# zyddnys/sd_animation_optical_flow

Hardware: AMD Instinct MI355X
Metric: frame-pairs/sec (flow+warp+mask) at 512x768 (higher is better)
Workload: dtype f32

## Files before the change

include/ofx.h:

```cpp
#ifndef OFX_H
#define OFX_H

#include <stddef.h>
#include <stdint.h>

#ifdef __cplusplus
extern "C" {
#endif

#define OFX_VERSION 100

#define OFX_EINVAL   (-1)
#define OFX_EALIGN   (-2)
#define OFX_ENOMEM   (-3)
#define OFX_EKEY     (-4)
#define OFX_ENODEV   (-5)

int ofx_version(void);
const char* ofx_error_string(int code);

int ofx_prof_enable(int on);
int ofx_prof_collect(char* json_out, size_t cap);

#define OFX_WARP_BILINEAR  0
// ... 101 lines not shown
int ofx_clip_embed(const int32_t* ids, const float* tok, const float* pos, float* out, int ldo, long rows, int T, int C, int vocab,
                   void* stream);
int ofx_quick_gelu(const float* x, int ldx, float* out, int ldo, long rows, int n, void* stream);

typedef struct ofx_ddim_coef {
    float cfg, sqrt_at, sqrt_1m_at, sqrt_aprev, dir_coef, sigma_t, g, sa, s1;
} ofx_ddim_coef;
#define OFX_DDIM_STEP       0
#define OFX_DDIM_BLEND_ONLY 1
int ofx_ddim_step(const float* x, int ldx, const float* eps_c, const float* eps_u, int lde, const float* guidance, int ldg,
                  const float* gmap, const float* step_noise, int ldsn, const float* init, int ldi, const float* nmask, int ldm,
                  const float* blend_noise, int ldbn, float* out0, int ldo0, float* out1, int ldo1, float* pred_out, int ldp,
                  const ofx_ddim_coef* coef, int mode, long rows, int C, void* stream);

size_t ofx_detect_edges_scratch_bytes(int B, int H, int W);
int ofx_detect_edges(const uint8_t* frames_bgr, uint8_t* edges, void* scratch, size_t scratch_bytes, int B, int H,
                     int W, int ksize, void* stream);
size_t ofx_canny_u8_scratch_bytes(int B, int H, int W);
int ofx_canny_u8(const uint8_t* images, int channels, uint8_t* edges, void* scratch, size_t scratch_bytes, int B, int H,
                 int W, int low, int high, void* stream);
int ofx_abs_diff_sum_u8(const uint8_t* a, long a_bstride, const uint8_t* b, long b_bstride,
                        unsigned long long* sums, int B, long n, void* stream);

#define OFX_ACT_NONE    0
#define OFX_ACT_RELU    1
#define OFX_ACT_SIGMOID 2
#define OFX_ACT_TANH    3

#define OFX_EPI_PLAIN   0
#define OFX_EPI_GRU_ZR  1
#define OFX_EPI_GRU_Q   2
#define OFX_EPI_FLOW    3

#define OFX_PREC_FP32   0
#define OFX_PREC_BF16X3 1
#define OFX_PREC_BF16X3_W 2
#define OFX_PREC_BF16X6_W 4
#define OFX_PREC_BF16X6 3
#define OFX_PREC_F16 5
#define OFX_PREC_F16_EPI (OFX_PREC_F16 | 256)

typedef struct ofx_conv_desc {
    const float* in0; int ld0; int c0;
    const float* in1; int ld1; int c1;
    const float* w;
    const float* scale;
    const float* shift;
    float* out; int ldo;
    const float* res; int ldres;
    const float* nmean; const float* nrstd;
    const float* addend; int ldadd;
    float* aux_z; float* aux_rh; float* aux_h; int ldh;
    float* aux_coords; float* aux_flow4;
    long a_zs, w_zs, o_zs; int nz;
    int B, Hin, Win, Hout, Wout, Cout, KH, KW, stride, padH, padW;
    int act, epi;
    int tile;
    int precision;
    void* splitk_ws;
    size_t splitk_ws_bytes;
    const float* wino_w;
    const float* wino4_w;
} ofx_conv_desc;
#define OFX_CONV_TILE_WINOGRAD 1
#define OFX_CONV_TILE_WINOGRAD4 2

int ofx_conv2d(const ofx_conv_desc* d, void* stream);
typedef struct ofx_conv_plan {
    int path;
    int bm, bn, wm, wn, bk;
    int prec;
    int ks;
    int ksplit;
    int mode;
    int mtiles, ntiles, group_m;
    int stats_rows;
} ofx_conv_plan;
int ofx_conv2d_plan(const ofx_conv_desc* d, size_t stats_cap_floats, int want_pool, ofx_conv_plan* out);
long ofx_pack_conv_weight(const float* w_oihw, int Cout, int Cin, int KH, int KW, int cin_pad,
                          float* out);
int ofx_split_conv_weight(const float* packed, long n_floats, float* out);
long ofx_wino_conv_weight(const float* w_oihw, int Cout, int Cin, float* out);
long ofx_wino15_conv_weight(const float* w_oihw, int Cout, int Cin, int KH, int KW, float* out);
long ofx_wino44_conv_weight(const float* w_oihw, int Cout, int Cin, float* out);
int ofx_split_conv_weight3(const float* packed, long n_floats, float* out);

int ofx_inorm_stats(const float* x, int ld, float* mean, float* rstd, float* scratch,
                    int B, long HW, int C, float eps, void* stream);
int ofx_conv2d_stats(const ofx_conv_desc* d, float* part, size_t part_floats, int* rows_per_image, void* stream);
int ofx_inorm_finalize(const float* part, float* mean, float* rstd, int B, int rows, long HW, int C, float eps, void* stream);
int ofx_inorm_apply(const float* x, const float* mean, const float* rstd, const float* res,
                    const float* res_mean, const float* res_rstd, float* out, int B, long HW, int C,
                    int relu, void* stream);
int ofx_preprocess_u8(const uint8_t* img, float* out, long npix, int bgr, void* stream);

int ofx_corr_slice_floats(int h_l, int w_l);
int ofx_corr_volume(const float* f1, const float* f2, float* const* pyr, int B, int h, int w, int D,
                    int levels, void* stream);
int ofx_corr_volume_split(const float* f1, const float* f2, float* const* pyr, int B, int h, int w, int D,
                          int levels, int planes, int shared_f2, void* stream);
int ofx_corr_lookup(const float* const* pyr, const float* coords, float* out, int ldo, int B, int h,
                    int w, int levels, int radius, void* stream);
int ofx_local_corr_fwd(const float* fmap1, const float* fmap2, const float* coords, float* corr,
                       int B, int H1, int W1, int H2, int W2, int C, int N, int r, void* stream);
int ofx_local_corr_bwd(const float* fmap1, const float* fmap2, const float* coords, const float* corr_grad,
                       float* fmap1_grad, float* fmap2_grad, int B, int H1, int W1, int H2, int W2, int C, int N,
                       int r, void* stream);
int ofx_local_corr_rows(const float* fmap1, const float* const* fmap2_levels, const int* idx1, const int* idx2,
                        const float* coords, float* rows, int ld, int B, int H1, int W1, int C, int levels, int radius,
                        int tiled, void* stream);
int ofx_avgpool2_nhwc(const float* in, float* out, int B, int H, int W, int C, void* stream);

int ofx_upsample_flow(const float* coords1, const float* mask, float* flow_up, int B, int h, int w,
                      void* stream);
int ofx_upsample_flow_warp(const float* coords1, const float* mask, float* flow_up, const uint8_t* frame,
                           uint8_t* warped, int B, int h, int w, float sign, void* stream);
int ofx_upflow8(const float* coords1, float* flow_up, int B, int h, int w, void* stream);
int ofx_upflow8_warp(const float* coords1, float* flow_up, const uint8_t* frame, uint8_t* warped, int B, int h, int w,
                     float sign, void* stream);
int ofx_flow_head(const float* x, int ldx, const float* w, int kpad, const float* bias, float* coords1, float* hx_flow,
                  int ldh, float* frows, int B, int h, int w_, void* stream);

size_t ofx_forward_interpolate_scratch_bytes(int B, int h, int w);
int ofx_forward_interpolate(const float* flow, float* out, void* scratch, size_t scratch_bytes, int B, int h, int w, void* stream);

typedef struct ofx_tensor {
    const char* name;
    const float* data;
    int ndim; long shape[4];
} ofx_tensor;

typedef struct ofx_raft ofx_raft;

int ofx_raft_create(const ofx_tensor* tensors, int n, ofx_raft** out);
int ofx_raft_destroy(ofx_raft* r);
size_t ofx_raft_workspace_bytes(const ofx_raft* r, int B, int H, int W);
size_t ofx_raft_workspace_bytes_mode(const ofx_raft* r, int n_images, int B, int H, int W, int flags);

#define OFX_RAFT_BGR          1
#define OFX_RAFT_SHARED_IMG2  2
#define OFX_RAFT_SHARED_IMG1  4
#define OFX_RAFT_ALT_CORR     8
#define OFX_RAFT_BF16X3      16
#define OFX_RAFT_BF16X6      64
#define OFX_RAFT_BN_BATCH   128
#define OFX_RAFT_SEPARATE_STATS 256
#define OFX_RAFT_VOL_BF16X3  512
#define OFX_RAFT_VOL_BF16X6 1024
#define OFX_RAFT_SERIAL       32
#define OFX_RAFT_FLOW_INIT  2048
#define OFX_RAFT_F16 4096

int ofx_raft_forward(ofx_raft* r, const uint8_t* image1, const uint8_t* image2, int B, int H, int W,
                     int iters, int flags, float* flow_up, float* flow_low, void* workspace,
                     size_t workspace_bytes, void* stream);
int ofx_raft_forward_warp(ofx_raft* r, const uint8_t* image1, const uint8_t* image2, int B, int H, int W,
                          int iters, int flags, float* flow_up, float* flow_low, const uint8_t* warp_frame,
                          float warp_sign, uint8_t* warped, void* workspace, size_t workspace_bytes, void* stream);
size_t ofx_raft_workspace_bytes_pairs(const ofx_raft* r, int n_images, int B, int H, int W);
int ofx_raft_forward_pairs(ofx_raft* r, const uint8_t* images, int n_images, const int* idx1,
                           const int* idx2, int B, int H, int W, int iters, int flags, float* flow_up,
                           float* flow_low, void* workspace, size_t workspace_bytes, void* stream);
int ofx_raft_forward_pairs_warp(ofx_raft* r, const uint8_t* images, int n_images, const int* idx1,
                                const int* idx2, int B, int H, int W, int iters, int flags, float* flow_up,
                                float* flow_low, const uint8_t* warp_frame, float warp_sign, int n_warp,
                                uint8_t* warped, void* workspace, size_t workspace_bytes, void* stream);
// ... 8 lines not shown
```

sd_animation_optical_flow_amd/_lib.py:

```python
from __future__ import annotations

import ctypes as C
import os

_HERE = os.path.dirname(os.path.abspath(__file__))
LIB_PATH = os.environ.get("OFX_LIB_PATH") or os.path.join(_HERE, "libofx.so")


class OfxLibraryError(RuntimeError):
    pass


class OfxError(RuntimeError):
    def __init__(self, code: int, where: str):
        self.code = code
        super().__init__(f"{where}: {error_string(code)} (code {code})")


class ConvDesc(C.Structure):
    _fields_ = [
        ("in0", C.c_void_p), ("ld0", C.c_int), ("c0", C.c_int),
        ("in1", C.c_void_p), ("ld1", C.c_int), ("c1", C.c_int),
        ("w", C.c_void_p), ("scale", C.c_void_p), ("shift", C.c_void_p),
        ("out", C.c_void_p), ("ldo", C.c_int),
        ("res", C.c_void_p), ("ldres", C.c_int),
        ("nmean", C.c_void_p), ("nrstd", C.c_void_p),
        ("addend", C.c_void_p), ("ldadd", C.c_int),
        ("aux_z", C.c_void_p), ("aux_rh", C.c_void_p), ("aux_h", C.c_void_p), ("ldh", C.c_int),
        ("aux_coords", C.c_void_p), ("aux_flow4", C.c_void_p),
        ("a_zs", C.c_long), ("w_zs", C.c_long), ("o_zs", C.c_long), ("nz", C.c_int),
        ("B", C.c_int), ("Hin", C.c_int), ("Win", C.c_int), ("Hout", C.c_int), ("Wout", C.c_int),
        ("Cout", C.c_int), ("KH", C.c_int), ("KW", C.c_int), ("stride", C.c_int),
        ("padH", C.c_int), ("padW", C.c_int),
        ("act", C.c_int), ("epi", C.c_int), ("tile", C.c_int), ("precision", C.c_int),
        ("splitk_ws", C.c_void_p), ("splitk_ws_bytes", C.c_size_t),
        ("wino_w", C.c_void_p),
        ("wino4_w", C.c_void_p),
    ]


class ConvPlan(C.Structure):
    _fields_ = [(n, C.c_int) for n in ("path", "bm", "bn", "wm", "wn", "bk", "prec", "ks", "ksplit", "mode", "mtiles", "ntiles",
                                       "group_m", "stats_rows")]


class MaskRoute(C.Structure):
    _fields_ = [(n, C.c_int) for n in ("kernel", "band_rows", "threads", "nplanes", "xcd_map", "lds_bytes", "workgroups")]


class DdimCoef(C.Structure):
    _fields_ = [(n, C.c_float) for n in ("cfg", "sqrt_at", "sqrt_1m_at", "sqrt_aprev", "dir_coef", "sigma_t", "g", "sa", "s1")]


class Tensor(C.Structure):
    _fields_ = [("name", C.c_char_p), ("data", C.c_void_p), ("ndim", C.c_int), ("shape", C.c_long * 4)]


_p, _i, _l, _f, _z = C.c_void_p, C.c_int, C.c_long, C.c_float, C.c_size_t

SIGNATURES = {
    "ofx_version": (_i, []),
    "ofx_error_string": (C.c_char_p, [_i]),
    "ofx_prof_enable": (_i, [_i]),
    "ofx_prof_collect": (_i, [C.c_char_p, _z]),
    "ofx_warp_u8": (_i, [_p, _l, _p, _p, _i, _i, _i, _i, _i, _f, _p]),
    "ofx_warp_f32": (_i, [_p, _l, _p, _p, _i, _i, _i, _i, _i, _f, _p]),
    "ofx_resize_cubic_f32": (_i, [_p, _p, _i, _i, _i, _i, _i, _i, _p]),
    "ofx_generate_mask": (_i, [_p, _p, _p, _i, _i, _i, _f, _i, _i, _p]),
    "ofx_dilate_u8": (_i, [_p, _p, _i, _i, _i, _i, _p]),
    "ofx_expand_mask": (_i, [_p, _p, _p, _p, _i, _i, _i, _i, _i, _p]),
    "ofx_mask_plan": (_i, [_i, _i, _i, _i, _i, _i, C.POINTER(MaskRoute)]),
    "ofx_travel_distance": (_i, [_p, _p, _p, _i, _i, _i, _f, _p]),
    "ofx_flow_magnitude": (_i, [_p, _p, _l, _p]),
    "ofx_travel_mask": (_i, [_p, _p, _p, _p, _p, _p, _i, _i, _i, _f, _i, _p]),
    "ofx_merge_images": (_i, [_p, _p, _p, _p, _i, _i, _i, _i, _p]),
    "ofx_mix_frames": (_i, [_p, _p, _p, _p, _i, _i, _i, _i, _f, _p]),
    "ofx_conf_sum": (_i, [_p, _p, _i, _l, _i, _i, _p]),
    "ofx_fb_confidence": (_i, [_p, _p, _p, _p, _i, _i, _i, _f, _p]),
    "ofx_warp_and_mask": (_i, [_p, _l, _p, _p, _p, _p, _i, _i, _i, _i, _i, _f, _f, _i, _i, _p]),
    "ofx_compose_scratch_bytes": (_z, [_i, _i, _i]),
    "ofx_compose_refs": (_i, [_p] * 9 + [_z, _i, _i, _i, _f, _i, _i, _p]),
    "ofx_conv2d": (_i, [C.POINTER(ConvDesc), _p]),
    "ofx_conv2d_plan": (_i, [C.POINTER(ConvDesc), _z, _i, C.POINTER(ConvPlan)]),
    "ofx_pack_conv_weight": (_l, [_p, _i, _i, _i, _i, _i, _p]),
    "ofx_wino_conv_weight": (_l, [_p, _i, _i, _p]),
    "ofx_wino15_conv_weight": (_l, [_p, _i, _i, _i, _i, _p]),
    "ofx_wino44_conv_weight": (_l, [_p, _i, _i, _p]),
    "ofx_split_conv_weight": (_i, [_p, _l, _p]),
    "ofx_split_conv_weight3": (_i, [_p, _l, _p]),
    "ofx_gaussian_blur_u8": (_i, [_p, _p, _p, _i, _i, _i, _f, _p]),
    "ofx_resize_bicubic_u8": (_i, [_p, _p, _p, _i, _i, _i, _i, _i, _p]),
    "ofx_sd_handoff": (_i, [_p] * 9 + [_i] * 5 + [_p]),
    "ofx_gaussian_blur_rgba_u8": (_i, [_p, _p, _p, _i, _i, _i, _f, _p]),
    "ofx_fill_mask_input_scratch_bytes": (_z, [_i, _i, _i]),
    "ofx_fill_mask_input": (_i, [_p, _p, _p, _p, _i, _i, _i, _p]),
    "ofx_detect_edges_scratch_bytes": (_z, [_i, _i, _i]),
    "ofx_detect_edges": (_i, [_p, _p, _p, _z, _i, _i, _i, _i, _p]),
    "ofx_canny_u8_scratch_bytes": (_z, [_i, _i, _i]),
    "ofx_canny_u8": (_i, [_p, _i, _p, _p, _z, _i, _i, _i, _i, _i, _p]),
    "ofx_abs_diff_sum_u8": (_i, [_p, _l, _p, _l, _p, _i, _l, _p]),
    "ofx_inorm_stats": (_i, [_p, _i, _p, _p, _p, _i, _l, _i, _f, _p]),
    "ofx_conv2d_stats": (_i, [C.POINTER(ConvDesc), _p, _z, _p, _p]),
    "ofx_inorm_finalize": (_i, [_p, _p, _p, _i, _i, _l, _i, _f, _p]),
    "ofx_inorm_apply": (_i, [_p, _p, _p, _p, _p, _p, _p, _i, _l, _i, _i, _p]),
    "ofx_preprocess_u8": (_i, [_p, _p, _l, _i, _p]),
    "ofx_groupnorm_scratch_bytes": (C.c_size_t, [_i, _i]),
    "ofx_groupnorm": (_i, [_p, _p, _p, _p, _p, C.c_size_t, _i, C.c_long, _i, _i, C.c_float, _i, _p]),
    "ofx_softmax_rows": (_i, [_p, C.c_long, C.c_long, _i, C.c_float, _p, C.c_long, C.c_long, _p]),
    "ofx_attention_workspace_bytes": (C.c_size_t, [_i, _i, _i, _i]),
    "ofx_attention_f32": (_i, [_p, _p, _p, _p, C.c_long, _p, _i, _i, _i, _i, C.c_float, _p, C.c_size_t, _p]),
    "ofx_attention_prec": (_i, [_p, _p, _p, _p, C.c_long, _p, _i, _i, _i, _i, C.c_float, _i, _p, C.c_size_t, _p]),
    "ofx_layernorm": (_i, [_p, _i, _p, _p, _p, _i, _i, _i, _f, _p]),
    "ofx_geglu": (_i, [_p, _i, _p, _i, _i, _i, _p]),
    "ofx_attention_bnhd_f32": (_i, [_p, _i, _p, _i, _p, _i, _p, _l, _p, _i, _i, _i, _i, _i, _i, _f, _p]),
    "ofx_attention_bnhd_prec": (_i, [_p, _i, _p, _i, _p, _i, _p, _l, _p, _i, _i, _i, _i, _i, _i, _f, _i, _p]),
    "ofx_upconv2x_weight": (_l, [_p, _i, _i, _p]),
    "ofx_upconv2x": (_i, [_p, _p, _p, _p, _i, _i, _i, _i, _i, _i, _p]),
    "ofx_upsample2x_nearest_f32": (_i, [_p, _p, _i, _i, _i, _i, _p]),
    "ofx_decode_to_u8": (_i, [_p, _i, _p, _i, _i, _i, _p]),
    "ofx_groupnorm_cat_scratch_bytes": (_z, [_i, _i]),
    "ofx_groupnorm_cat": (_i, [_p, _i, _i, _p, _i, _i, _p, _i, _p, _p, _p, _p, _z, _i, _l, _i, _f, _i, _p]),
    "ofx_emb_linear": (_i, [_p, _i, _p, _p, _p, _i, _i, _i, _i, _i, _p]),
    "ofx_timestep_embedding": (_i, [_p, _p, _p, _i, _i, _p]),
    "ofx_ddim_step": (_i, [_p, _i, _p, _p, _i, _p, _i, _p, _p, _i, _p, _i, _p, _i, _p, _i, _p, _i, _p, _i, _p, _i, C.POINTER(DdimCoef), _i, _l, _i, _p]),
    "ofx_conv3x3_silu": (_i, [_p, _i, _i, _p, _i, _p, _p, _i, _i, _i, _i, _i, _i, _i, _p]),
    "ofx_clip_embed": (_i, [_p, _p, _p, _p, _i, _l, _i, _i, _i, _p]),
    "ofx_quick_gelu": (_i, [_p, _i, _p, _i, _l, _i, _p]),
    "ofx_corr_slice_floats": (_i, [_i, _i]),
    "ofx_corr_volume": (_i, [_p, _p, C.POINTER(_p), _i, _i, _i, _i, _i, _p]),
    "ofx_corr_volume_split": (_i, [_p, _p, C.POINTER(_p), _i, _i, _i, _i, _i, _i, _i, _p]),
    "ofx_corr_lookup": (_i, [C.POINTER(_p), _p, _p, _i, _i, _i, _i, _i, _i, _p]),
    "ofx_local_corr_fwd": (_i, [_p, _p, _p, _p, _i, _i, _i, _i, _i, _i, _i, _i, _p]),
    "ofx_local_corr_bwd": (_i, [_p] * 6 + [_i] * 8 + [_p]),
    "ofx_local_corr_rows": (_i, [_p] * 6 + [_i] * 8 + [_p]),
    "ofx_avgpool2_nhwc": (_i, [_p, _p, _i, _i, _i, _i, _p]),
    "ofx_upsample_flow": (_i, [_p, _p, _p, _i, _i, _i, _p]),
    "ofx_upsample_flow_warp": (_i, [_p, _p, _p, _p, _p, _i, _i, _i, _f, _p]),
    "ofx_upflow8": (_i, [_p, _p, _i, _i, _i, _p]),
    "ofx_upflow8_warp": (_i, [_p, _p, _p, _p, _i, _i, _i, _f, _p]),
    "ofx_flow_head": (_i, [_p, _i, _p, _i, _p, _p, _p, _i, _p, _i, _i, _i, _p]),
    "ofx_forward_interpolate_scratch_bytes": (_z, [_i, _i, _i]),
    "ofx_forward_interpolate": (_i, [_p, _p, _p, _z, _i, _i, _i, _p]),
    "ofx_raft_create": (_i, [C.POINTER(Tensor), _i, C.POINTER(_p)]),
    "ofx_raft_destroy": (_i, [_p]),
    "ofx_raft_workspace_bytes": (_z, [_p, _i, _i, _i]),
    "ofx_raft_workspace_bytes_mode": (_z, [_p, _i, _i, _i, _i, _i]),
    "ofx_raft_forward": (_i, [_p, _p, _p, _i, _i, _i, _i, _i, _p, _p, _p, _z, _p]),
    "ofx_raft_forward_warp": (_i, [_p, _p, _p, _i, _i, _i, _i, _i, _p, _p, _p, _f, _p, _p, _z, _p]),
    "ofx_raft_workspace_bytes_pairs": (_z, [_p, _i, _i, _i, _i]),
    "ofx_raft_forward_pairs": (_i, [_p, _p, _i, C.POINTER(_i), C.POINTER(_i), _i, _i, _i, _i, _i, _p, _p, _p, _z, _p]),
    "ofx_raft_forward_pairs_warp": (_i, [_p, _p, _i, C.POINTER(_i), C.POINTER(_i), _i, _i, _i, _i, _i, _p, _p, _p, _f, _i, _p, _p, _z, _p]),
    "ofx_raft_variant": (_i, [_p]),
    "ofx_raft_buffer": (_i, [_p, C.c_char_p, C.POINTER(_p), C.POINTER(_z)]),
}

_lib = None


def lib() -> C.CDLL:
    global _lib
    if _lib is not None:
        return _lib
    if not os.path.exists(LIB_PATH):
        raise OfxLibraryError(
            f"{LIB_PATH} not found: the HIP library has not been built. There is no CPU fallback; "
            "run `python -c 'import __graft_entry__ as g; g.build()'` at the repo root.")
    try:
        handle = C.CDLL(LIB_PATH)
    except OSError as e:
# ... 20 lines not shown
```

sd_animation_optical_flow_amd/csrc/conv_wino.hip:

```cpp
#include "ofx_internal.h"

#include <cmath>
#include <cstdlib>
#include <cstring>

namespace {

constexpr int kWBK = 16;
constexpr int kLDV = kWBK + 4;
constexpr int kOOB = 0x7FFFFFF0;

template <int W_, int H_, int Y0, int X0> struct HaloGeom {
    static constexpr int W = W_, H = H_, y_org = Y0, x_org = X0;
    static constexpr int pix = W * H;
    static constexpr int items = pix * (kWBK / 4);
    static constexpr int slots = (items + 255) / 256;
};
template <bool VERT> struct Halo15 : HaloGeom<VERT ? 16 : 20, VERT ? 12 : 8, VERT ? -2 : 0, VERT ? 0 : -2> {
    static constexpr int ldh = VERT ? 16 : 20;
    static constexpr int floats = Halo15::pix * ldh;
    __device__ static int at(int pix) { return pix * ldh; }
};
struct Halo3x3 : HaloGeom<18, 10, -1, -1> {
    static constexpr int lpair = 36, lrow = 336;
    static constexpr int floats = H * lrow;
    __device__ static int at(int y, int x) { return y * lrow + (x >> 1) * lpair + (x & 1) * 16; }
    __device__ static int at(int pix) { return at(pix / W, pix % W); }
};

struct WinoK {
    const float* in0;
    const float* in1;
    const float* u;
    const float* scale;
    const float* shift;
    const float* addend;
    const float* res;
    const float* nmean;
    const float* nrstd;
    float* stats;
    float* out;
    float* aux_z;
    float* aux_rh;
    float* aux_h;
    int ld0, c0, ld1, cin, ldo, ldadd, ldh, ldres;
    int H, W, Cout, act;
    int nblk;
    int nb32;
    int tpr, tpi, mtiles;
    int bytes0, bytes1, bytesu;
    float alpha;
    int vec4;
};

struct Patch {
    int nb, pb, y0, x0;
};

template <int PH = 8, int PW = 16> __device__ __forceinline__ Patch wino_patch(const WinoK& p) {
    const int nblk = p.mtiles * p.nblk;
    const int bid = blockIdx.x;
    const int q8 = nblk >> 3, r8 = nblk & 7;
    const int xcd = bid & 7, idx = bid >> 3;
    const int L = (xcd < r8 ? xcd * (q8 + 1) : r8 * (q8 + 1) + (xcd - r8) * q8) + idx;
    const int nb = L % p.nblk, mt = L / p.nblk;
    const int pb = mt / p.tpi;
    const int trem = mt - pb * p.tpi;
    const int py = trem / p.tpr;
    return {nb, pb, py * PH, (trem - py * p.tpr) * PW};
}

typedef int v4i __attribute__((ext_vector_type(4)));

template <class HALO, bool NORM> struct HaloStage {
    const WinoK& p;
    const int pb, tid;
    const float* in1s;
    int bytes1s;
    int hpix[HALO::slots];
    unsigned hok = 0;
    int hq;
    struct Regs {
        float4 pa[HALO::slots];
        float4 pmu, prs;
    } own;

    __device__ __forceinline__ HaloStage(const WinoK& p_, const Patch& pt, int tid_) : p(p_), pb(pt.pb), tid(tid_) {
        in1s = p.in1 ? p.in1 : p.in0;
        bytes1s = p.in1 ? p.bytes1 : p.bytes0;
#pragma unroll
        for (int k = 0; k < HALO::slots; ++k) {
            const int i = tid + 256 * k;
            const int pix = i >> 2;
            const int hy = pix / HALO::W, hx = pix - hy * HALO::W;
            const int gy = pt.y0 + HALO::y_org + hy, gx = pt.x0 + HALO::x_org + hx;
            const bool ok = i < HALO::items && (unsigned)gy < (unsigned)p.H && (unsigned)gx < (unsigned)p.W;
            hpix[k] = ok ? (pt.pb * p.H + gy) * p.W + gx : 0;
            hok |= (ok ? 1u : 0u) << k;
        }
        hq = (tid & 3) * 16;
    }
    __device__ __forceinline__ void issue(int cb) { issue(cb, own); }
    __device__ __forceinline__ void store(float* Hs) const { store(Hs, own); }
    __device__ __forceinline__ void issue(int cb, Regs& r) {
        const int c = cb * kWBK;
        const bool s0 = c < p.c0;
        const __amdgpu_buffer_rsrc_t rs = __builtin_amdgcn_make_buffer_rsrc((void*)(s0 ? p.in0 : in1s), (short)0, s0 ? p.bytes0 : bytes1s, 0x00020000);
        const int so = (s0 ? c : c - p.c0) * 4;
        const int ldb = (s0 ? p.ld0 : p.ld1) * 4;
#pragma unroll
        for (int k = 0; k < HALO::slots; ++k) {
            const int vo = ((hok >> k) & 1u) ? hpix[k] * ldb + hq : kOOB;
            v4i t = __builtin_amdgcn_raw_buffer_load_b128(rs, vo, so, 0);
            r.pa[k] = *reinterpret_cast<float4*>(&t);
        }
        if constexpr (NORM) {
            const long at = (long)pb * p.c0 + c + (tid & 3) * 4;
            r.pmu = *reinterpret_cast<const float4*>(p.nmean + at);
            r.prs = *reinterpret_cast<const float4*>(p.nrstd + at);
        }
    }
    __device__ __forceinline__ void store(float* Hs, const Regs& r) const {
#pragma unroll
        for (int k = 0; k < HALO::slots; ++k) {
            const int i = tid + 256 * k;
            if (HALO::slots * 256 > HALO::items && k == HALO::slots - 1 && i >= HALO::items) break;
            float4 v = r.pa[k];
            if constexpr (NORM) {
                v.x = fmaxf((v.x - r.pmu.x) * r.prs.x, 0.f);
                v.y = fmaxf((v.y - r.pmu.y) * r.prs.y, 0.f);
                v.z = fmaxf((v.z - r.pmu.z) * r.prs.z, 0.f);
                v.w = fmaxf((v.w - r.pmu.w) * r.prs.w, 0.f);
                if (!((hok >> k) & 1u)) v = make_float4(0.f, 0.f, 0.f, 0.f);
            }
            *reinterpret_cast<float4*>(&Hs[HALO::at(i >> 2) + (i & 3) * 4]) = v;
// ... 271 lines not shown
            const int tile = (e & 3) + 8 * (e >> 2) + 4 * (lane >> 5);
            const float m0 = acc[0][nt][e], m1 = acc[1][nt][e], m2 = acc[2][nt][e], m3 = acc[3][nt][e];
            X[((wave * 2 + 0) * 32 + tile) * kLDX + (lane & 31)] = m0 + m1 + m2;
            X[((wave * 2 + 1) * 32 + tile) * kLDX + (lane & 31)] = m1 - m2 - m3;
        }
        __syncthreads();
        const int oc = pt.nb * 64 + nt * 32 + on;
        if (oc < p.Cout) {
            const float sc = (p.scale ? p.scale[oc] : 1.0f) * p.alpha;
            const float sh = p.shift ? p.shift[oc] : 0.0f;
            float st_s = 0.0f, st_q = 0.0f;
#pragma unroll
            for (int ty = 0; ty < 4; ++ty) {
                const int tile = ty * 8 + otx;
                float x[4][2];
#pragma unroll
                for (int w = 0; w < 4; ++w)
#pragma unroll
                    for (int j = 0; j < 2; ++j) x[w][j] = X[((w * 2 + j) * 32 + tile) * kLDX + on];
                float r[2][2];
                if constexpr (RES) {
#pragma unroll
                    for (int a = 0; a < 2; ++a)
#pragma unroll
                        for (int j = 0; j < 2; ++j)
                            r[a][j] = p.res[(((long)pt.pb * p.H + pt.y0 + 2 * ty + a) * p.W + pt.x0 + 2 * otx + j) * p.ldres + oc];
                }
#pragma unroll
                for (int a = 0; a < 2; ++a)
#pragma unroll
                    for (int j = 0; j < 2; ++j) {
                        const float y = a == 0 ? x[0][j] + x[1][j] + x[2][j] : x[1][j] - x[2][j] - x[3][j];
                        const long pix = ((long)pt.pb * p.H + pt.y0 + 2 * ty + a) * p.W + pt.x0 + 2 * otx + j;
                        float v = fmaxf(y * sc + sh, act_lo);
                        if constexpr (RES) v = fmaxf(v + r[a][j], 0.0f);
                        p.out[pix * p.ldo + oc] = v;
                        if constexpr (STATS) {
                            st_s += v;
                            st_q = fmaf(v, v, st_q);
                        }
                    }
            }
            if constexpr (STATS) {
                st_s += __shfl_xor(st_s, 32, 64);
                st_q += __shfl_xor(st_q, 32, 64);
                if (lane < 32) {
                    Sx[((nt * 4 + wave) * 32 + on) * 2 + 0] = st_s;
                    Sx[((nt * 4 + wave) * 32 + on) * 2 + 1] = st_q;
                }
            }
        }
    }
    if constexpr (STATS) {
        __syncthreads();
        const int nt = tid >> 5;
        const int oc = pt.nb * 64 + nt * 32 + on;
        if (tid < 64 && oc < p.Cout) {
            float s = 0.0f, q = 0.0f;
#pragma unroll
            for (int w = 0; w < 4; ++w) {
                s += Sx[((nt * 4 + w) * 32 + on) * 2 + 0];
                q += Sx[((nt * 4 + w) * 32 + on) * 2 + 1];
            }
            const long row = (long)pt.pb * p.tpi + (pt.y0 >> 3) * p.tpr + (pt.x0 >> 4);
            p.stats[(row * p.Cout + oc) * 2 + 0] = s;
            p.stats[(row * p.Cout + oc) * 2 + 1] = q;
        }
    }
}

template <bool VERT, int EPI>
__global__ __launch_bounds__(256, 2) void wino15_conv_kernel(const WinoK p) {
    using T = Wino15<VERT>;
    using HALO = typename T::HALO;
    __shared__ __attribute__((aligned(16))) float smem[HALO::floats + 8 * 32 * kLDV];
    float* const Hs = smem;
    float* const Vs = smem + HALO::floats;
    const int tid = threadIdx.x, lane = tid & 63;
    const int wave = __builtin_amdgcn_readfirstlane(tid >> 6);
    const Patch pt = wino_patch(p);
    f32x16 acc[8][1];
    wino_slabs_staged<T>(p, pt, Hs, Vs, tid, wave, acc);

    const int n = pt.nb * 128 + wave * 32 + (lane & 31);
    if (n >= p.Cout) return;
    const float sc = (p.scale ? p.scale[n] : 1.0f) * p.alpha;
    const float sh = p.shift ? p.shift[n] : 0.0f;
    const float act_lo = p.act == OFX_ACT_RELU ? 0.0f : -3.402823466e38f;
    const int hd = p.Cout >> 1;
    const bool r_half = EPI == OFX_EPI_GRU_ZR && pt.nb * 128 >= hd;
#pragma unroll
    for (int eb = 0; eb < 16; eb += 4) {
        long pix[4][4];
        float y[4][4], ad[4][4], x1[4][4], x2[4][4];
#pragma unroll
        for (int u = 0; u < 4; ++u) {
            const int e = eb + u;
            const int tile = (e & 3) + 8 * (e >> 2) + 4 * (lane >> 5);
#pragma unroll
            for (int i = 0; i < 4; ++i) pix[u][i] = ((long)pt.pb * p.H + pt.y0 + T::oy(tile, i)) * p.W + pt.x0 + T::ox(tile, i);
            const float m0 = acc[0][0][e], m1 = acc[1][0][e], m2 = acc[2][0][e], m3 = acc[3][0][e];
            const float m4 = acc[4][0][e], m5 = acc[5][0][e], m6 = acc[6][0][e], m7 = acc[7][0][e];
            const float s12 = m1 + m2, d12 = m1 - m2, s34 = m3 + m4, d34 = m3 - m4, s56 = m5 + m6, d56 = m5 - m6;
            y[u][0] = m0 + s12 + s34 + s56;
            y[u][1] = d12 + 2.0f * d34 + 0.5f * d56;
            y[u][2] = s12 + 4.0f * s34 + 0.25f * s56;
            y[u][3] = d12 + 8.0f * d34 + 0.125f * d56 + m7;
        }
#pragma unroll
        for (int u = 0; u < 4; ++u)
#pragma unroll
            for (int i = 0; i < 4; ++i) {
                ad[u][i] = p.addend ? p.addend[pix[u][i] * p.ldadd + n] : 0.0f;
                x1[u][i] = EPI == OFX_EPI_GRU_ZR ? (r_half ? p.aux_h[pix[u][i] * p.ldh + n - hd] : 1.0f)
                           : EPI == OFX_EPI_GRU_Q ? p.aux_z[pix[u][i] * p.Cout + n] : 0.0f;
                x2[u][i] = EPI == OFX_EPI_GRU_Q ? p.aux_h[pix[u][i] * p.ldh + n] : 0.0f;
            }
#pragma unroll
        for (int u = 0; u < 4; ++u)
#pragma unroll
            for (int i = 0; i < 4; ++i) {
                const float v = y[u][i] * sc + sh + ad[u][i];
                if (EPI == OFX_EPI_PLAIN) {
                    p.out[pix[u][i] * p.ldo + n] = fmaxf(v, act_lo);
                } else if (EPI == OFX_EPI_GRU_ZR) {
                    const float g = ofx_sigmoid(v) * x1[u][i];
                    if (r_half) p.aux_rh[pix[u][i] * hd + n - hd] = g;
                    else p.aux_z[pix[u][i] * hd + n] = g;
                } else {
                    p.aux_h[pix[u][i] * p.ldh + n] = (1.0f - x1[u][i]) * x2[u][i] + x1[u][i] * ofx_tanh(v);
                }
            }
    }
}

struct Halo44 {
    static constexpr int W = 34, H = 18;
    static constexpr int lquad = 34, lrow = 308;
    static constexpr int floats = H * lrow;
    static constexpr int items = W * H * 2;
    static constexpr int threads = 768;
    static constexpr int slots = (items + threads - 1) / threads;
    __device__ __host__ static constexpr int at(int y, int x) { return y * lrow + (x >> 2) * lquad + (x & 3) * 8; }
    static constexpr int ltrow = 336;
    static constexpr int tfloats = 6 * 4 * ltrow;
    static constexpr int titems = 4 * W * 4;
};
constexpr int kLDX4 = 40;
constexpr int kXF4 = 12 * 4 * 16 * kLDX4;
constexpr int kStage44 = 2 * (Halo44::floats + Halo44::tfloats);
constexpr int kSmem44 = (kStage44 > kXF4 ? kStage44 : kXF4) * 4;
constexpr int kNorm44 = kSmem44 / 4 - kStage44;
constexpr int kNorm44MaxCin = kNorm44 / 2 / kWBK * kWBK;
constexpr int kSX4 = 2 * 48 * 32 * 2;
static_assert(kNorm44 >= 0 && kSX4 <= kXF4, "the fused options live in the plain kernel's LDS");

__global__ __launch_bounds__(768, 1) void wino44_conv_kernel(const WinoK p) {
    extern __shared__ __attribute__((aligned(16))) float smem44[];
    constexpr bool NORM = false, RES = false, STATS = false;
#include "conv_wino44_body.inl"
}

template <bool NORM, bool RES, bool STATS>
__global__ __launch_bounds__(768, 1) void wino44_fused_kernel(const WinoK p) {
    extern __shared__ __attribute__((aligned(16))) float smem44[];
#include "conv_wino44_body.inl"
}


using WinoKernel = void (*)(WinoK);

const WinoKernel kKernels22[8] = {wino_conv_kernel<false, false, false>, wino_conv_kernel<false, false, true>,
                                  wino_conv_kernel<false, true, false>,  nullptr,
                                  wino_conv_kernel<true, false, false>,  wino_conv_kernel<true, false, true>,
                                  wino_conv_kernel<true, true, false>,   nullptr};
const WinoKernel kKernels15[8] = {wino15_conv_kernel<true, OFX_EPI_PLAIN>,  wino15_conv_kernel<true, OFX_EPI_GRU_ZR>,
                                  wino15_conv_kernel<true, OFX_EPI_GRU_Q>,  wino15_conv_kernel<false, OFX_EPI_PLAIN>,
                                  wino15_conv_kernel<false, OFX_EPI_GRU_ZR>, wino15_conv_kernel<false, OFX_EPI_GRU_Q>,
                                  nullptr,                                  nullptr};
const WinoKernel kKernels44[8] = {wino44_conv_kernel,                       wino44_fused_kernel<false, false, true>,
                                  wino44_fused_kernel<false, true, false>,  nullptr,
                                  wino44_fused_kernel<true, false, false>,  wino44_fused_kernel<true, false, true>,
                                  wino44_fused_kernel<true, true, false>,   nullptr};

struct WinoAlg {
    bool one_d;
    int ph, pw;
    int points, outputs;
    int cblk;
    int threads, dyn_lds;
    const float* ofx_conv_desc::*u;
    int tile;
    long min_grid;
    bool per_block;
    bool gates;
    bool norm_pair;
    int norm_max_cin;
    int path, path_fused;
    const WinoKernel* kernels;
};

const WinoAlg kAlgs[] = {
    {false, 16, 32, 36, 16, 64, 768, kSmem44, &ofx_conv_desc::wino4_w, OFX_CONV_TILE_WINOGRAD4, 768, true,
     false, true, kNorm44MaxCin, kPathWino44, kPathWino44Fused, kKernels44},
    {false, 8, 16, 16, 4, 64, 256, 0, &ofx_conv_desc::wino_w, OFX_CONV_TILE_WINOGRAD, 1024, true,
     false, false, 0x7FFFFFFF, kPathWino3x3, kPathWino3x3, kKernels22},
    {true, 8, 16, 8, 4, 128, 256, 0, &ofx_conv_desc::wino_w, OFX_CONV_TILE_WINOGRAD, 256, false,
     true, false, 0, kPathWino15, kPathWino15, kKernels15},
};
constexpr int kNumAlgs = sizeof kAlgs / sizeof kAlgs[0];

bool is_1d(int KH, int KW) { return (KH == 1 && KW == 5) || (KH == 5 && KW == 1); }

bool wino_fits(const WinoAlg& a, const ofx_conv_desc* d) {
    const int cin = d->c0 + d->c1;
    const float* const u = d->*a.u;
    const bool plain = d->epi == OFX_EPI_PLAIN && d->out != nullptr && d->ldo >= d->Cout && (d->act == OFX_ACT_NONE || d->act == OFX_ACT_RELU);
    const bool shape = a.one_d ? is_1d(d->KH, d->KW) : d->KH == 3 && d->KW == 3;
    bool epi;
    if (a.gates) {
        epi = !d->nmean && !d->res && (plain || (d->epi == OFX_EPI_GRU_ZR && (d->Cout / 2) % a.cblk == 0) || d->epi == OFX_EPI_GRU_Q);
    } else {
        epi = plain && !d->addend && (!d->res || d->ldres >= d->Cout) && (!a.norm_pair || (d->nmean != nullptr) == (d->nrstd != nullptr)) &&
              (!d->nmean || (d->nrstd && !d->in1 && d->c0 <= a.norm_max_cin && ofx_aligned16(d->nmean) && ofx_aligned16(d->nrstd)));
    }
    return shape && epi && d->padH == d->KH / 2 && d->padW == d->KW / 2 && d->precision == OFX_PREC_FP32 && d->nz <= 1 && d->stride == 1 &&
           d->Hout == d->Hin && d->Wout == d->Win && d->Hin % a.ph == 0 && d->Win % a.pw == 0 && cin % kWBK == 0 && d->c0 % kWBK == 0 &&
           u != nullptr && ofx_aligned16(u);
}

int wino_stats_rows(const WinoAlg& a, const ofx_conv_desc* d) {
    return !a.gates && d->act == OFX_ACT_NONE && !d->res ? (d->Hin / a.ph) * (d->Win / a.pw) : 0;
}

int wino_args(const WinoAlg& a, const ofx_conv_desc* d, float alpha, float* stats, WinoK* out) {
    WinoK k{};
    k.in0 = d->in0; k.in1 = d->in1; k.u = d->*a.u; k.scale = d->scale; k.shift = d->shift; k.addend = d->addend; k.out = d->out;
    k.res = d->res; k.nmean = d->nmean; k.nrstd = d->nrstd; k.stats = stats;
    k.aux_z = d->aux_z; k.aux_rh = d->aux_rh; k.aux_h = d->aux_h;
    k.ld0 = d->ld0; k.c0 = d->c0; k.ld1 = d->ld1; k.cin = d->c0 + d->c1; k.ldo = d->ldo; k.ldadd = d->ldadd; k.ldh = d->ldh;
    k.ldres = d->ldres;
    k.H = d->Hin; k.W = d->Win; k.Cout = d->Cout; k.act = d->act;
    k.nblk = (d->Cout + a.cblk - 1) / a.cblk;
    k.nb32 = a.cblk / 32 * k.nblk;
    k.tpr = d->Win / a.pw;
    k.tpi = (d->Hin / a.ph) * k.tpr;
    const long mtiles = (long)d->B * k.tpi;
    const long npix = (long)d->B * d->Hin * d->Win;
    const long ext0 = ((npix - 1) * d->ld0 + d->c0) * 4, ext1 = d->in1 ? ((npix - 1) * d->ld1 + d->c1) * 4 : 0;
    const long extu = (long)a.points * k.nb32 * 32 * k.cin * 4;
    OFX_REQUIRE(ext0 < (1L << 31) - 64 && ext1 < (1L << 31) - 64 && extu < (1L << 31) - 64, OFX_EINVAL);
    OFX_REQUIRE(mtiles * k.nblk < (1L << 31) && (a.one_d || npix * d->ldo < (1L << 31)), OFX_EINVAL);
    k.mtiles = (int)mtiles;
    k.bytes0 = (int)ext0; k.bytes1 = (int)ext1; k.bytesu = (int)extu;
    k.alpha = alpha;
    k.vec4 = ofx_aligned16(d->out) && d->ldo % 4 == 0 && ofx_aligned16(d->scale) && ofx_aligned16(d->shift) &&
             (!d->res || (ofx_aligned16(d->res) && d->ldres % 4 == 0));
    *out = k;
    return 0;
}

int wino_launch_kernel(const WinoAlg& a, int v, const WinoK& k, hipStream_t s, hipEvent_t stop_event) {
    const WinoKernel kernel = v >= 0 && v < 8 ? a.kernels[v] : nullptr;
    OFX_REQUIRE(kernel != nullptr, OFX_EINVAL);
    if (a.dyn_lds > 65536) {
        static bool allowed[64][kNumAlgs][8] = {};
        int dev = 0;
        if (hipGetDevice(&dev) != hipSuccess || dev < 0 || dev >= 64) return OFX_EINVAL;
        bool& ok = allowed[dev][&a - kAlgs][v];
        if (!ok) {
            const hipError_t e = hipFuncSetAttribute(reinterpret_cast<const void*>(kernel), hipFuncAttributeMaxDynamicSharedMemorySize, a.dyn_lds);
            if (e != hipSuccess) return (int)e;
            ok = true;
        }
    }
    const dim3 grid((unsigned)(k.mtiles * k.nblk), 1, 1), block(a.threads, 1, 1);
    if (stop_event) hipExtLaunchKernelGGL(kernel, grid, block, a.dyn_lds, s, nullptr, stop_event, 0, k);
    else hipLaunchKernelGGL(kernel, grid, block, a.dyn_lds, s, k);
    return ofx_launch_status();
}

}

int ofx_conv_wino_choose(const ofx_conv_desc* d, bool want_stats, size_t stats_cap, bool pool, bool no_wino, bool no_wino15, bool no_wino44,
                         OfxWinoChoice* c) {
    *c = OfxWinoChoice{};
    const bool off[kNumAlgs] = {no_wino44, no_wino, no_wino15};
    const bool one_d = is_1d(d->KH, d->KW);
    for (int i = 0; i < kNumAlgs; ++i) {
        const WinoAlg& a = kAlgs[i];
        const bool force = d->tile == a.tile;
        if (a.one_d != one_d || !(force || (d->tile == 0 && !off[i] && d->*a.u))) continue;
        const int srows = want_stats ? wino_stats_rows(a, d) : 0;
        const bool stats_ok = !want_stats || (srows > 0 && (size_t)d->B * srows * d->Cout * 2 <= stats_cap);
        if (!(stats_ok && !pool && wino_fits(a, d))) continue;
        const long patches = (long)d->B * (d->Hin / a.ph) * (d->Win / a.pw);
        if (!force && patches * (a.per_block ? (d->Cout + a.cblk - 1) / a.cblk : 1) < a.min_grid) continue;
        c->path = want_stats || d->res || d->nmean || d->nrstd ? a.path_fused : a.path;
        c->stats_rows = srows;
        c->flops = 2.0 * a.points * ((double)d->B * d->Hout * d->Wout / a.outputs) * (double)(d->c0 + d->c1) * d->Cout;
        return 0;
    }
    return d->tile == OFX_CONV_TILE_WINOGRAD || d->tile == OFX_CONV_TILE_WINOGRAD4 ? OFX_EINVAL : 0;
}

int ofx_conv_wino_launch(const ofx_conv_desc* d, int path, float alpha, float* stats, hipStream_t s, hipEvent_t stop_event) {
    const WinoAlg* a = nullptr;
    for (const WinoAlg& row : kAlgs)
        if (path == row.path || path == row.path_fused) a = &row;
    OFX_REQUIRE(a && (!stats || wino_stats_rows(*a, d) > 0), OFX_EINVAL);
    WinoK k;
    if (int st = wino_args(*a, d, alpha, stats, &k)) return st;
    const int v = a->gates ? (d->epi >= OFX_EPI_PLAIN && d->epi <= OFX_EPI_GRU_Q ? (d->KH == 5 ? 0 : 3) + d->epi : -1)
                           : (k.nmean ? 4 : 0) | (k.res ? 2 : 0) | (k.stats ? 1 : 0);
    return wino_launch_kernel(*a, v, k, s, stop_event);
}

namespace {

template <class XF>
long wino_weight(const float* w, int Cout, int Cin, int taps, int points, int cblk, float* out, XF xf) {
    OFX_REQUIRE(Cout > 0 && Cin > 0 && Cin % kWBK == 0, OFX_EINVAL);
    const int nb32 = cblk / 32 * ((Cout + cblk - 1) / cblk);
    const long n = (long)points * nb32 * 32 * Cin;
    if (!out) return n;
    OFX_REQUIRE(w != nullptr, OFX_EINVAL);
    std::memset(out, 0, (size_t)n * sizeof(float));
    double u[16];
    for (int o = 0; o < Cout; ++o)
        for (int c = 0; c < Cin; ++c) {
            xf(w + ((size_t)o * Cin + c) * taps, u);
            for (int q = 0; q < points; ++q) {
                const long at = ((((long)q * nb32 + o / 32) * (Cin / 8) + c / 8) * 2 + (c % 8) / 4) * 128 + 4 * (o % 32) + c % 4;
                out[at] = (float)u[q];
            }
        }
    return n;
}

}

extern "C" long ofx_wino_conv_weight(const float* w, int Cout, int Cin, float* out) {
    return wino_weight(w, Cout, Cin, 9, 16, 64, out, [](const float* g, double* u) {
        static const double G[4][3] = {{1, 0, 0}, {0.5, 0.5, 0.5}, {0.5, -0.5, 0.5}, {0, 0, 1}};
        double gg[4][3];
        for (int i = 0; i < 4; ++i)
            for (int x = 0; x < 3; ++x) gg[i][x] = G[i][0] * g[x] + G[i][1] * g[3 + x] + G[i][2] * g[6 + x];
        for (int i = 0; i < 4; ++i)
            for (int j = 0; j < 4; ++j) u[4 * i + j] = gg[i][0] * G[j][0] + gg[i][1] * G[j][1] + gg[i][2] * G[j][2];
    });
}

extern "C" long ofx_wino15_conv_weight(const float* w, int Cout, int Cin, int KH, int KW, float* out) {
    OFX_REQUIRE(is_1d(KH, KW), OFX_EINVAL);
    return wino_weight(w, Cout, Cin, 5, 8, 128, out, [](const float* g, double* u) {
        static const double G[8][5] = {
            {1, 0, 0, 0, 0},
            {-2.0 / 9, -2.0 / 9, -2.0 / 9, -2.0 / 9, -2.0 / 9},
            {-2.0 / 9, 2.0 / 9, -2.0 / 9, 2.0 / 9, -2.0 / 9},
            {1.0 / 90, 1.0 / 45, 2.0 / 45, 4.0 / 45, 8.0 / 45},
            {1.0 / 90, -1.0 / 45, 2.0 / 45, -4.0 / 45, 8.0 / 45},
            {32.0 / 45, 16.0 / 45, 8.0 / 45, 4.0 / 45, 2.0 / 45},
            {32.0 / 45, -16.0 / 45, 8.0 / 45, -4.0 / 45, 2.0 / 45},
            {0, 0, 0, 0, 1},
        };
        for (int q = 0; q < 8; ++q) {
            u[q] = 0.0;
            for (int t = 0; t < 5; ++t) u[q] += G[q][t] * (double)g[t];
        }
    });
}

extern "C" long ofx_wino44_conv_weight(const float* w, int Cout, int Cin, float* out) {
    OFX_REQUIRE(Cout > 0 && Cin > 0 && Cin % kWBK == 0, OFX_EINVAL);
    const int nb32 = 2 * ((Cout + 63) / 64);
    const long n = 36L * nb32 * 32 * Cin;
    if (!out) return n;
    OFX_REQUIRE(w != nullptr, OFX_EINVAL);
    std::memset(out, 0, (size_t)n * sizeof(float));
    static const double G[6][3] = {{1.0 / 4, 0, 0},           {-1.0 / 6, -1.0 / 6, -1.0 / 6}, {-1.0 / 6, 1.0 / 6, -1.0 / 6},
                                   {1.0 / 24, 1.0 / 12, 1.0 / 6}, {1.0 / 24, -1.0 / 12, 1.0 / 6}, {0, 0, 1}};
    for (int o = 0; o < Cout; ++o)
        for (int c = 0; c < Cin; ++c) {
            const float* g = w + ((size_t)o * Cin + c) * 9;
            double gg[6][3];
            for (int i = 0; i < 6; ++i)
                for (int x = 0; x < 3; ++x) gg[i][x] = G[i][0] * g[x] + G[i][1] * g[3 + x] + G[i][2] * g[6 + x];
            for (int i = 0; i < 6; ++i)
                for (int j = 0; j < 6; ++j) {
                    const double u = gg[i][0] * G[j][0] + gg[i][1] * G[j][1] + gg[i][2] * G[j][2];
                    const long q = 6 * i + j;
                    const long at = ((((q * nb32 + o / 32) * (Cin / 8) + c / 8) * 2 + (c % 4) / 2) * 2 + (c % 8) / 4) * 64 + 2 * (o % 32) + c % 2;
                    out[at] = (float)u;
                }
        }
    return n;
}
```

Baseline: 373.9.

## Transpose wino15 gated epilogue through LDS for vectorized float4 channel stores

The Winograd 1x5/5x1 gated-conv epilogue (plain, GRU z/r, GRU q) used to have each lane write one channel to scattered pixels with scalar loads and stores. It now stages each wave's output tile through LDS so every lane holds four consecutive channels of one pixel, then does float4 loads of addend and aux tensors and float4 stores. A host-side alignment check picks the vector path and keeps a scalar tail for partial quads. This should cut memory transactions on the epilogue, at the cost of LDS traffic, wave barriers and extra code complexity.

```diff
diff --git a/include/ofx.h b/include/ofx.h
--- a/include/ofx.h
+++ b/include/ofx.h
@@ -207,6 +207,7 @@
 int ofx_split_conv_weight(const float* packed, long n_floats, float* out);
 long ofx_wino_conv_weight(const float* w_oihw, int Cout, int Cin, float* out);
 long ofx_wino15_conv_weight(const float* w_oihw, int Cout, int Cin, int KH, int KW, float* out);
+int ofx_conv_wino15_vec(const ofx_conv_desc* d);
 long ofx_wino44_conv_weight(const float* w_oihw, int Cout, int Cin, float* out);
 int ofx_split_conv_weight3(const float* packed, long n_floats, float* out);
 
diff --git a/sd_animation_optical_flow_amd/_lib.py b/sd_animation_optical_flow_amd/_lib.py
--- a/sd_animation_optical_flow_amd/_lib.py
+++ b/sd_animation_optical_flow_amd/_lib.py
@@ -85,6 +85,7 @@
     "ofx_pack_conv_weight": (_l, [_p, _i, _i, _i, _i, _i, _p]),
     "ofx_wino_conv_weight": (_l, [_p, _i, _i, _p]),
     "ofx_wino15_conv_weight": (_l, [_p, _i, _i, _i, _i, _p]),
+    "ofx_conv_wino15_vec": (_i, [C.POINTER(ConvDesc)]),
     "ofx_wino44_conv_weight": (_l, [_p, _i, _i, _p]),
     "ofx_split_conv_weight": (_i, [_p, _l, _p]),
     "ofx_split_conv_weight3": (_i, [_p, _l, _p]),
diff --git a/sd_animation_optical_flow_amd/csrc/conv_wino.hip b/sd_animation_optical_flow_amd/csrc/conv_wino.hip
--- a/sd_animation_optical_flow_amd/csrc/conv_wino.hip
+++ b/sd_animation_optical_flow_amd/csrc/conv_wino.hip
@@ -1,8 +1,10 @@
 #include "ofx_internal.h"
 
+#include <algorithm>
 #include <cmath>
 #include <cstdlib>
 #include <cstring>
+#include <type_traits>
 
 namespace {
 
@@ -51,6 +53,7 @@
     int bytes0, bytes1, bytesu;
     float alpha;
     int vec4;
+    int vec15;
 };
 
 struct Patch {
@@ -488,56 +491,142 @@
     f32x16 acc[8][1];
     wino_slabs_staged<T>(p, pt, Hs, Vs, tid, wave, acc);
 
-    const int n = pt.nb * 128 + wave * 32 + (lane & 31);
-    if (n >= p.Cout) return;
-    const float sc = (p.scale ? p.scale[n] : 1.0f) * p.alpha;
-    const float sh = p.shift ? p.shift[n] : 0.0f;
     const float act_lo = p.act == OFX_ACT_RELU ? 0.0f : -3.402823466e38f;
     const int hd = p.Cout >> 1;
     const bool r_half = EPI == OFX_EPI_GRU_ZR && pt.nb * 128 >= hd;
-#pragma unroll
-    for (int eb = 0; eb < 16; eb += 4) {
-        long pix[4][4];
-        float y[4][4], ad[4][4], x1[4][4], x2[4][4];
+    const int cq = lane & 7, ps = lane >> 3;
+    const int nw0 = pt.nb * 128 + wave * 32;
+    const int nv = p.Cout - (nw0 + 4 * cq);
+    const bool all_quads = p.vec15 && nw0 + 32 <= p.Cout;
+    const bool quad = p.vec15 && nv >= 4;
+    float sc[4], sh[4];
+    if (quad) {
+        const float4 s4 = p.scale ? *reinterpret_cast<const float4*>(p.scale + nw0 + 4 * cq) : make_float4(1.0f, 1.0f, 1.0f, 1.0f);
+        const float4 h4 = p.shift ? *reinterpret_cast<const float4*>(p.shift + nw0 + 4 * cq) : make_float4(0.0f, 0.0f, 0.0f, 0.0f);
+        sc[0] = s4.x, sc[1] = s4.y, sc[2] = s4.z, sc[3] = s4.w;
+        sh[0] = h4.x, sh[1] = h4.y, sh[2] = h4.z, sh[3] = h4.w;
+    } else {
+#pragma unroll
+        for (int c = 0; c < 4; ++c) {
+            sc[c] = p.scale && c < nv ? p.scale[nw0 + 4 * cq + c] : 1.0f;
+            sh[c] = p.shift && c < nv ? p.shift[nw0 + 4 * cq + c] : 0.0f;
+        }
+    }
+#pragma unroll
+    for (int c = 0; c < 4; ++c) sc[c] *= p.alpha;
+    typedef float v4f __attribute__((ext_vector_type(4)));
+    typedef __attribute__((address_space(1))) char gchar;
+    typedef __attribute__((address_space(1))) float gfloat;
+    typedef __attribute__((address_space(1))) v4f gv4f;
+    auto gbase = [](const void* base) __attribute__((always_inline)) {
+        unsigned long b = reinterpret_cast<unsigned long>(base);
+        asm volatile("" : "+s"(b));
+        return (gchar*)b;
+    };
+    auto ld4 = [&](auto all, const void* base, unsigned off, float fill, float (&v)[4]) __attribute__((always_inline)) {
+        gchar* const g = gbase(base);
+        v[0] = v[1] = v[2] = v[3] = fill;
+        if (decltype(all)::value || quad) {
+            const v4f t = *(const gv4f*)(g + off);
+            v[0] = t.x, v[1] = t.y, v[2] = t.z, v[3] = t.w;
+        } else if (nv > 0) {
+            const gfloat* const q = (const gfloat*)(g + off);
+            v[0] = q[0];
+            if (nv > 1) {
+                v[1] = q[1];
+                if (nv > 2) {
+                    v[2] = q[2];
+                    if (nv > 3) v[3] = q[3];
+                }
+            }
+        }
+    };
+    auto st4 = [&](auto all, void* base, unsigned off, const float (&v)[4]) __attribute__((always_inline)) {
+        gchar* const g = gbase(base);
+        if (decltype(all)::value || quad) {
+            *(gv4f*)(g + off) = v4f{v[0], v[1], v[2], v[3]};
+        } else if (nv > 0) {
+            gfloat* const q = (gfloat*)(g + off);
+            q[0] = v[0];
+            if (nv > 1) {
+                q[1] = v[1];
+                if (nv > 2) {
+                    q[2] = v[2];
+                    if (nv > 3) q[3] = v[3];
+                }
+            }
+        }
+    };
+    const long pix0 = ((long)pt.pb * p.H + pt.y0) * p.W + pt.x0;
+    const int ld_x1 = EPI == OFX_EPI_GRU_Q ? p.Cout : p.ldh;
+    const int ld_d = EPI == OFX_EPI_PLAIN ? p.ldo : EPI == OFX_EPI_GRU_ZR ? hd : p.ldh;
+    const float* const b_ad = p.addend ? p.addend + pix0 * p.ldadd + nw0 : nullptr;
+    const float* const b_x1 = EPI == OFX_EPI_GRU_Q ? p.aux_z + pix0 * p.Cout + nw0 : r_half ? p.aux_h + pix0 * p.ldh + (nw0 - hd) : nullptr;
+    const float* const b_x2 = EPI == OFX_EPI_GRU_Q ? p.aux_h + pix0 * p.ldh + nw0 : nullptr;
+    float* const b_d = EPI == OFX_EPI_PLAIN    ? p.out + pix0 * p.ldo + nw0
+                       : EPI == OFX_EPI_GRU_ZR ? (r_half ? p.aux_rh + pix0 * hd + (nw0 - hd) : p.aux_z + pix0 * hd + nw0)
+                                               : p.aux_h + pix0 * p.ldh + nw0;
+    const unsigned o_ad = (unsigned)(ps * p.ldadd + 4 * cq) * 4u, o_x1 = (unsigned)(ps * ld_x1 + 4 * cq) * 4u;
+    const unsigned o_x2 = (unsigned)(ps * p.ldh + 4 * cq) * 4u, o_d = (unsigned)(ps * ld_d + 4 * cq) * 4u;
+    float* const X = smem + wave * (32 * 32);
+    float* const xw = X + (VERT ? 4 : 16) * (lane >> 5) * 32 + (lane & 31);
+    const float* const xr = X + ps * 32 + 4 * cq;
+    __syncthreads();
+    auto passes = [&](auto all) __attribute__((always_inline)) {
+#pragma unroll
+    for (int k = 0; k < 4; ++k) {
 #pragma unroll
         for (int u = 0; u < 4; ++u) {
-            const int e = eb + u;
-            const int tile = (e & 3) + 8 * (e >> 2) + 4 * (lane >> 5);
-#pragma unroll
-            for (int i = 0; i < 4; ++i) pix[u][i] = ((long)pt.pb * p.H + pt.y0 + T::oy(tile, i)) * p.W + pt.x0 + T::ox(tile, i);
+            const int e = 4 * k + u;
             const float m0 = acc[0][0][e], m1 = acc[1][0][e], m2 = acc[2][0][e], m3 = acc[3][0][e];
             const float m4 = acc[4][0][e], m5 = acc[5][0][e], m6 = acc[6][0][e], m7 = acc[7][0][e];
             const float s12 = m1 + m2, d12 = m1 - m2, s34 = m3 + m4, d34 = m3 - m4, s56 = m5 + m6, d56 = m5 - m6;
-            y[u][0] = m0 + s12 + s34 + s56;
-            y[u][1] = d12 + 2.0f * d34 + 0.5f * d56;
-            y[u][2] = s12 + 4.0f * s34 + 0.25f * s56;
-            y[u][3] = d12 + 8.0f * d34 + 0.125f * d56 + m7;
-        }
-#pragma unroll
-        for (int u = 0; u < 4; ++u)
-#pragma unroll
-            for (int i = 0; i < 4; ++i) {
-                ad[u][i] = p.addend ? p.addend[pix[u][i] * p.ldadd + n] : 0.0f;
-                x1[u][i] = EPI == OFX_EPI_GRU_ZR ? (r_half ? p.aux_h[pix[u][i] * p.ldh + n - hd] : 1.0f)
-                           : EPI == OFX_EPI_GRU_Q ? p.aux_z[pix[u][i] * p.Cout + n] : 0.0f;
-                x2[u][i] = EPI == OFX_EPI_GRU_Q ? p.aux_h[pix[u][i] * p.ldh + n] : 0.0f;
+            float y[4];
+            y[0] = m0 + s12 + s34 + s56;
+            y[1] = d12 + 2.0f * d34 + 0.5f * d56;
+            y[2] = s12 + 4.0f * s34 + 0.25f * s56;
+            y[3] = d12 + 8.0f * d34 + 0.125f * d56 + m7;
+#pragma unroll
+            for (int i = 0; i < 4; ++i) xw[(VERT ? 8 * i + u : 4 * u + i) * 32] = y[i];
+        }
+        __builtin_amdgcn_fence(__ATOMIC_RELEASE, "wavefront");
+        __builtin_amdgcn_wave_barrier();
+        __builtin_amdgcn_fence(__ATOMIC_ACQUIRE, "wavefront");
+        float yq[4][4], ad[4][4], x1[4][4], x2[4][4];
+        int dpix[4];
+#pragma unroll
+        for (int j = 0; j < 4; ++j) {
+            dpix[j] = VERT ? (4 * (k >> 1) + j) * p.W + 8 * (k & 1) : (2 * k + (j >> 1)) * p.W + 8 * (j & 1);
+            const float4 t = *reinterpret_cast<const float4*>(xr + 8 * j * 32);
+            yq[j][0] = t.x, yq[j][1] = t.y, yq[j][2] = t.z, yq[j][3] = t.w;
+        }
+#pragma unroll
+        for (int j = 0; j < 4; ++j) {
+            if (p.addend) ld4(all, b_ad + (long)dpix[j] * p.ldadd, o_ad, 0.0f, ad[j]);
+            else ad[j][0] = ad[j][1] = ad[j][2] = ad[j][3] = 0.0f;
+            if (EPI == OFX_EPI_GRU_Q || r_half) ld4(all, b_x1 + (long)dpix[j] * ld_x1, o_x1, 1.0f, x1[j]);
+            else x1[j][0] = x1[j][1] = x1[j][2] = x1[j][3] = 1.0f;
+            if (EPI == OFX_EPI_GRU_Q) ld4(all, b_x2 + (long)dpix[j] * p.ldh, o_x2, 0.0f, x2[j]);
+        }
+        __builtin_amdgcn_fence(__ATOMIC_RELEASE, "wavefront");
+        __builtin_amdgcn_wave_barrier();
+        __builtin_amdgcn_fence(__ATOMIC_ACQUIRE, "wavefront");
+#pragma unroll
+        for (int j = 0; j < 4; ++j) {
+            float o[4];
+#pragma unroll
+            for (int c = 0; c < 4; ++c) {
+                const float v = yq[j][c] * sc[c] + sh[c] + ad[j][c];
+                if (EPI == OFX_EPI_PLAIN) o[c] = fmaxf(v, act_lo);
+                else if (EPI == OFX_EPI_GRU_ZR) o[c] = ofx_sigmoid(v) * x1[j][c];
+                else o[c] = (1.0f - x1[j][c]) * x2[j][c] + x1[j][c] * ofx_tanh(v);
             }
-#pragma unroll
-        for (int u = 0; u < 4; ++u)
-#pragma unroll
-            for (int i = 0; i < 4; ++i) {
-                const float v = y[u][i] * sc + sh + ad[u][i];
-                if (EPI == OFX_EPI_PLAIN) {
-                    p.out[pix[u][i] * p.ldo + n] = fmaxf(v, act_lo);
-                } else if (EPI == OFX_EPI_GRU_ZR) {
-                    const float g = ofx_sigmoid(v) * x1[u][i];
-                    if (r_half) p.aux_rh[pix[u][i] * hd + n - hd] = g;
-                    else p.aux_z[pix[u][i] * hd + n] = g;
-                } else {
-                    p.aux_h[pix[u][i] * p.ldh + n] = (1.0f - x1[u][i]) * x2[u][i] + x1[u][i] * ofx_tanh(v);
-                }
-            }
-    }
+            st4(all, b_d + (long)dpix[j] * ld_d, o_d, o);
+        }
+    }
+    };
+    if (all_quads) passes(std::true_type{});
+    else passes(std::false_type{});
 }
 
 struct Halo44 {
@@ -637,6 +726,14 @@
 
 int wino_stats_rows(const WinoAlg& a, const ofx_conv_desc* d) {
     return !a.gates && d->act == OFX_ACT_NONE && !d->res ? (d->Hin / a.ph) * (d->Win / a.pw) : 0;
+}
+
+bool wino15_vec(const ofx_conv_desc* d) {
+    if (!(ofx_aligned16(d->scale) && ofx_aligned16(d->shift) && (!d->addend || (ofx_aligned16(d->addend) && d->ldadd % 4 == 0)))) return false;
+    if (d->epi == OFX_EPI_PLAIN) return ofx_aligned16(d->out) && d->ldo % 4 == 0;
+    const bool h = ofx_aligned16(d->aux_z) && ofx_aligned16(d->aux_h) && d->ldh % 4 == 0;
+    if (d->epi == OFX_EPI_GRU_ZR) return h && ofx_aligned16(d->aux_rh) && (d->Cout / 2) % 4 == 0;
+    return h && d->Cout % 4 == 0;
 }
 
 int wino_args(const WinoAlg& a, const ofx_conv_desc* d, float alpha, float* stats, WinoK* out) {
@@ -662,6 +759,11 @@
     k.alpha = alpha;
     k.vec4 = ofx_aligned16(d->out) && d->ldo % 4 == 0 && ofx_aligned16(d->scale) && ofx_aligned16(d->shift) &&
              (!d->res || (ofx_aligned16(d->res) && d->ldres % 4 == 0));
+    if (a.gates) {
+        const int ldmax = std::max(std::max(d->epi == OFX_EPI_PLAIN ? d->ldo : d->ldh, d->addend ? d->ldadd : 0), d->Cout);
+        OFX_REQUIRE(ldmax < (1 << 26), OFX_EINVAL);
+        k.vec15 = wino15_vec(d);
+    }
     *out = k;
     return 0;
 }
@@ -720,6 +822,17 @@
     const int v = a->gates ? (d->epi >= OFX_EPI_PLAIN && d->epi <= OFX_EPI_GRU_Q ? (d->KH == 5 ? 0 : 3) + d->epi : -1)
                            : (k.nmean ? 4 : 0) | (k.res ? 2 : 0) | (k.stats ? 1 : 0);
     return wino_launch_kernel(*a, v, k, s, stop_event);
+}
+
+extern "C" int ofx_conv_wino15_vec(const ofx_conv_desc* d) {
+    OFX_REQUIRE(d != nullptr, OFX_EINVAL);
+    const WinoAlg* a = nullptr;
+    for (const WinoAlg& row : kAlgs)
+        if (row.gates) a = &row;
+    OFX_REQUIRE(a && wino_fits(*a, d), OFX_EINVAL);
+    WinoK k;
+    if (int st = wino_args(*a, d, 1.0f, nullptr, &k)) return st;
+    return k.vec15;
 }
 
 namespace {
```

Result: no change. 376.8, median of 6 (+0.8%).
